# CleanDiffuserTeam/CleanDiffuser

Hardware: AMD Instinct MI355X
Metric: denoised trajectories/sec @ (B=256,H=32,D=23) 20-step DDIM (higher is better)
Workload: dtype f32; 1 GPU; BASELINE configs[1]: JannerUNet1d Diffuser H=32 D=23, 20-step DDIM, global B=256, whole DiscreteDiffusionSDE.sample() call as a pipeline makes it (initial draw inside); batch_per_gpu=256, global_batch=256, horizon=32, dim=23, sample_steps=20, world_size=1, parallelism=batch-sharded x1; the only data-path collective is the all-gather of the result

## Files before the change

### cleandiffuser_amd/csrc/cdx_unet2.hip

```cpp
#include <hip/hip_runtime.h>
#include <stdint.h>
#include <string.h>

#include "../../include/cdx.h"
#include "cdx_act.h"
#include "cdx_ops2.h"
#include "cdx_step.h"

typedef float f32x4 __attribute__((ext_vector_type(4)));
typedef const int __attribute__((address_space(4))) cint;
#pragma clang diagnostic push
#pragma clang diagnostic ignored "-Wold-style-cast"
static __device__ __forceinline__ const cint* as_const(const int* p) { return (const cint*)p; }
#pragma clang diagnostic pop

void cdx_set_err(const char* msg);

template <int NWV> struct WG {
    static constexpr int THREADS = NWV * 64;
    static constexpr int PF = NWV == 8 ? 8 : 16;
    static constexpr int OPW = CDX2_HDR_WORDS + NWV * CDX2_ITEM_WORDS;
};

namespace {
// ... 42 lines not shown
    switch (id) {
        case 2: return mish2(x);
        case 3: {
            const float z = fabsf(x) * 0.70710678118654752f;
            const float t = __builtin_amdgcn_rcpf(fmaf(0.3275911f, z, 1.0f));
            const float poly = t * fmaf(t, fmaf(t, fmaf(t, fmaf(t, 1.061405429f, -1.453152027f), 1.421413741f), -0.284496736f), 0.254829592f);
            return 0.5f * x * (1.0f + copysignf(1.0f - poly * __expf(-z * z), x));
        }
        case 4: return cdx_act_leaky(x);
        case 5: return cdx_act_silu(x);
        case 6: return cdx_act_relu(x);
        case 7: return 0.5f * x * (1.0f + tanhf(0.7978845608028654f * (x + 0.044715f * x * x * x)));
        case 9: return tanhf(x);
        default: return x;
    }
}

struct M16 {
    static constexpr int COLS = 16, KSTEP = 16;
    static __device__ __forceinline__ int col(int lane) { return lane & 15; }
    static __device__ __forceinline__ int koff(int lane) { return 4 * (lane >> 4); }
    static __device__ __forceinline__ int drow(int lane) { return 4 * (lane >> 4); }
    static __device__ __forceinline__ f32x4 mfma(float a, float b, f32x4 c) {
        return __builtin_amdgcn_mfma_f32_16x16x4f32(a, b, c, 0, 0, 0);
    }
};
struct M4 {
    static constexpr int COLS = 4, KSTEP = 4;
    static __device__ __forceinline__ int col(int lane) { return lane & 3; }
    static __device__ __forceinline__ int koff(int) { return 0; }
    static __device__ __forceinline__ int drow(int lane) { return 4 * (lane >> 2); }
    static __device__ __forceinline__ f32x4 mfma(float a, float b, f32x4 c) {
        return __builtin_amdgcn_mfma_f32_4x4x1f32(a, b, c, 0, 0, 0);
    }
};

typedef const cdx_unet2_launch __attribute__((address_space(4))) KArg;

#pragma clang diagnostic push
#pragma clang diagnostic ignored "-Wold-style-cast"
static __device__ __forceinline__ const KArg* kernarg() { return (const KArg*)__builtin_amdgcn_kernarg_segment_ptr(); }
#pragma clang diagnostic pop

struct Geom {
    int l_cols, cstride, ostride, sstride, stage;
    int gsh, grows;
};

struct Item { int woff, nq, tap, cc, part, col0, pad, ooff, src, sstr, ccn; };

__device__ __forceinline__ Item make_item(int woff, int nq, int tc, int part, int col0, int po, int ss, int ccn) {
    return Item{woff, nq, tc & 255, tc >> 8, part, col0, po & 255, po >> 8, ss & 0xffff, ss >> 16, ccn};
}
__device__ __forceinline__ Item load_item(const cint* it) {
    return make_item(it[CDX2_I2_WOFF], it[CDX2_I2_NQ], it[CDX2_I2_TAPCC], it[CDX2_I2_PART], it[CDX2_I2_COL0],
                     it[CDX2_I2_PADOOFF], it[CDX2_I2_SRCSTR], it[CDX2_I2_CCN]);
}

#define CDX2_DW(vd, k) __builtin_amdgcn_readlane((vd), (k))
template <int NWV>
__device__ __forceinline__ int load_desc(const int* __restrict__ ops, int op, int lane, int wave) {
    const int w = lane < CDX2_HDR_WORDS ? lane : CDX2_HDR_WORDS + wave * CDX2_ITEM_WORDS + (lane & (CDX2_ITEM_WORDS - 1));
    return ops[op * WG<NWV>::OPW + w];
}
__device__ __forceinline__ Item inline_item(int vd) {
    const int b = CDX2_HDR_WORDS;
    return make_item(CDX2_DW(vd, b + CDX2_I2_WOFF), CDX2_DW(vd, b + CDX2_I2_NQ), CDX2_DW(vd, b + CDX2_I2_TAPCC),
                     CDX2_DW(vd, b + CDX2_I2_PART), CDX2_DW(vd, b + CDX2_I2_COL0), CDX2_DW(vd, b + CDX2_I2_PADOOFF),
                     CDX2_DW(vd, b + CDX2_I2_SRCSTR), CDX2_DW(vd, b + CDX2_I2_CCN));
}

__device__ __forceinline__ void stamp(unsigned long long* slot, int tid) {
    if (slot && tid == 0) *slot = __builtin_amdgcn_s_memtime();
}

typedef unsigned u32x4 __attribute__((ext_vector_type(4)));
#define CDX2_N_CUS 256
#define CDX2_GETREG_XCC_ID ((3 << 11) | 20)
static __device__ __forceinline__ int mul24i(int a, int b) { return __mul24(a, b); }
static __device__ __forceinline__ int wave_of(int tid) { return __builtin_amdgcn_readfirstlane(tid >> 6); }
#pragma clang diagnostic push
#pragma clang diagnostic ignored "-Wold-style-cast"
struct WStream {
    __amdgpu_buffer_rsrc_t rs;
    int lane16;
    __device__ __forceinline__ WStream(const float* wblob, int lane)
        : rs(__builtin_amdgcn_make_buffer_rsrc((void*)wblob, 0, 0x7fffffff, 0x00020000)), lane16(lane * 16) {}
    __device__ __forceinline__ f32x4 load(int woff, int q) const {
        return __builtin_bit_cast(f32x4, __builtin_amdgcn_raw_buffer_load_b128(rs, lane16, woff * 4 + q * 1024, 0));
    }
};
#pragma clang diagnostic pop

template <int PF> struct Ring { f32x4 rec[PF]; };

template <class M, int NT, int T, int NWV, bool PROF, bool GRP = false>
__device__ __forceinline__ void conv_kloop(const Geom& g, const float* __restrict__ wblob, int vd, const cint* ops,
                                           Item it, int n_items, float* __restrict__ lds, int tf, int lane, int wave,
                                           Ring<WG<NWV>::PF>& ring, unsigned long long* prof, int tune) {
    constexpr int PF = WG<NWV>::PF, NW = NWV;
    constexpr int BD = NWV == 4 ? ((M::KSTEP == 4 && NT * T == 1) ? 8 : 4)
                                : (NT * T == 1 ? (M::KSTEP == 4 ? 8 : 4) : (NT * T == 2 ? 4 : 2));
    constexpr int NA = NWV == 4 ? 4 : ((M::KSTEP == 4 && NT == 1) ? 4 : 2);
    static_assert(PF % BD == 0, "operand ring must divide the weight ring");
    const int ptid = (wave == 0 && lane == 0) ? 0 : 1;
    for (int item = wave; item < n_items; item += NW) {
        if (item != wave) it = load_item(ops + CDX2_DW(vd, CDX2_W2_ITEMS) + (item - NW) * CDX2_ITEM_WORDS);
        const int nq = it.nq, ccn = it.ccn;
        int cc = it.cc;
        int cur[NT], tstep[NT], mcol[NT];
#pragma unroll
        for (int nt = 0; nt < NT; ++nt) {
            mcol[nt] = it.col0 + nt * M::COLS + M::col(lane);
            const bool valid = mcol[nt] < g.l_cols;
            int mrow = mul24i(mcol[nt], g.cstride);
            if (GRP && g.grows) mrow = mul24i(mcol[nt] >> g.gsh, g.grows) + mul24i(mcol[nt] & ((1 << g.gsh) - 1), g.cstride);
            const int row = valid ? mrow - it.pad + CDX2_HALO2 + it.tap : 0;
            cur[nt] = it.src + __mul24(row, it.sstr) + M::koff(lane) + cc * M::KSTEP;
            tstep[nt] = (valid ? it.sstr : 0) - ccn * M::KSTEP;
        }
        if (PROF && prof && item == 0) { asm volatile("" ::"s"(nq), "v"(cur[0])); stamp(prof + 4, ptid); }
        f32x4 acc[T][NT][NA];
#pragma unroll
        for (int t = 0; t < T; ++t)
#pragma unroll
            for (int nt = 0; nt < NT; ++nt)
#pragma unroll
                for (int j = 0; j < NA; ++j) acc[t][nt][j] = (f32x4){0.f, 0.f, 0.f, 0.f};

        const WStream ws(wblob, lane);
        const int woff = it.woff;
#define CDX2_WLOAD(q) ws.load(woff, (q))
        f32x4 wr[PF];
        if (item == wave) {
#pragma unroll
            for (int u = 0; u < PF; ++u) wr[u] = ring.rec[u];
        } else {
#pragma unroll
            for (int u = 0; u < PF; ++u) wr[u] = CDX2_WLOAD(u);
        }
        f32x4 bq[BD][T][NT];
        auto fetch = [&](f32x4 (&bv)[T][NT]) {
#pragma unroll
            for (int t = 0; t < T; ++t)
#pragma unroll
                for (int nt = 0; nt < NT; ++nt) bv[t][nt] = *reinterpret_cast<const f32x4*>(lds + t * tf + cur[nt]);
        };
        auto advance = [&]() {
#pragma unroll
            for (int nt = 0; nt < NT; ++nt) cur[nt] += M::KSTEP;
            if (++cc == ccn) {
                cc = 0;
#pragma unroll
                for (int nt = 0; nt < NT; ++nt) cur[nt] += tstep[nt];
            }
        };
        const bool aligned = (M::KSTEP == 4 || GRP) && (ccn % PF) == 0 && (it.cc % PF) == 0 && nq >= 2 * PF;
        if (aligned) {
#pragma unroll
            for (int j = 0; j < BD - 1; ++j)
// ... 43 lines not shown
                cc0 = wrap ? 0 : cc0 + PF;
#pragma unroll
                for (int nt = 0; nt < NT; ++nt) rbn[nt] = rb[nt] + PF * M::KSTEP * 4 + (wrap ? tstep[nt] * 4 : 0);
#pragma unroll
                for (int u = 0; u < PF; ++u) {
                    const int ua = u + BD - 1;
#pragma unroll
                    for (int t = 0; t < T; ++t)
#pragma unroll
                        for (int nt = 0; nt < NT; ++nt)
                            bq[ua % BD][t][nt] = *reinterpret_cast<const f32x4*>(
                                ldsb + (ua < PF ? rb[nt] : rbn[nt]) + t * tf * 4 + (ua % PF) * M::KSTEP * 4);
#pragma unroll
                    for (int j = 0; j < 4; ++j)
#pragma unroll
                        for (int t = 0; t < T; ++t)
#pragma unroll
                            for (int nt = 0; nt < NT; ++nt)
                                acc[t][nt][j % NA] = M::mfma(wr[u][j], bq[u % BD][t][nt][j], acc[t][nt][j % NA]);
                    if (u > 0) refill(u - 1, qi + u - 1 + PF);
                    else if (qi > 0) refill(PF - 1, qi - 1 + PF);
                    if (NWV == 4 || T >= 2) __builtin_amdgcn_sched_barrier(0);
                }
#pragma unroll
                for (int nt = 0; nt < NT; ++nt) rb[nt] = rbn[nt];
            }
            cc = cc0 + BD - 2;
#pragma unroll
            for (int nt = 0; nt < NT; ++nt) cur[nt] = rb[nt] / 4 + (BD - 2) * M::KSTEP;
        }
        for (; qi < nq; qi += PF) {
#pragma unroll
            for (int u = 0; u < PF; ++u) {
                if (qi + u >= nq) break;
                chunk(wr[u], u, qi + u + BD - 1 < nq);
                const int q = qi + u - 1 + PF;
                if (q >= PF && q < nq) refill((u + PF - 1) % PF, q);
            }
        }
        if (NWV == 8) __builtin_amdgcn_s_setprio(0);
        if (PROF && prof && item == 0) { asm volatile("" ::"v"(acc[0][0][0][0]), "v"(acc[0][0][1][0])); stamp(prof + 6, ptid); }
#pragma unroll
        for (int t = 0; t < T; ++t)
#pragma unroll
            for (int nt = 0; nt < NT; ++nt) {
                if (mcol[nt] < g.l_cols) {
                    const int n = mul24i(mcol[nt], g.ostride) + it.ooff;
                    f32x4 dd = acc[t][nt][0];
                    if (NA == 2) dd += acc[t][nt][NA - 1];
                    if (NA == 4) dd = (acc[t][nt][0] + acc[t][nt][1]) + (acc[t][nt][NA / 2] + acc[t][nt][NA - 1]);
                    *reinterpret_cast<f32x4*>(lds + t * tf + g.stage + it.part + mul24i(n, g.sstride) + M::drow(lane)) = dd;
                }
            }
    }
}

struct EpiDesc {
    int flags, c_out, l_out, coutp, sstride, ksplit, dst, dstride, res, rstride, shift, nk;
    int save, savestr, stats, dst2, d2stride;
    int kpost;
    float inv_cnt;
    float odiv;
    int cgreal4;
};
template <bool BWD>
__device__ __forceinline__ EpiDesc decode_epi(int vd) {
    EpiDesc e;
    e.flags = CDX2_DW(vd, CDX2_W2_FLAGS); e.c_out = CDX2_DW(vd, CDX2_W2_COUT); e.l_out = CDX2_DW(vd, CDX2_W2_LOUT);
    e.coutp = CDX2_DW(vd, CDX2_W2_COUTP); e.sstride = CDX2_DW(vd, CDX2_W2_SSTRIDE); e.ksplit = CDX2_DW(vd, CDX2_W2_KSPLIT);
    e.dst = CDX2_DW(vd, CDX2_W2_DST); e.dstride = CDX2_DW(vd, CDX2_W2_DST_STRIDE); e.res = CDX2_DW(vd, CDX2_W2_RES);
    e.rstride = CDX2_DW(vd, CDX2_W2_RES_STRIDE); e.shift = CDX2_DW(vd, CDX2_W2_CG4_SHIFT); e.nk = CDX2_DW(vd, CDX2_W2_NK);
    e.inv_cnt = __int_as_float(CDX2_DW(vd, CDX2_W2_INV_CNT));
    e.kpost = CDX2_DW(vd, CDX2_W2_KPOST);
    e.odiv = BWD ? 1.0f : __int_as_float(CDX2_DW(vd, CDX2_W2_ODIV));
    e.cgreal4 = BWD ? 0 : CDX2_DW(vd, CDX2_W2_CGREAL4);
    e.save = e.savestr = e.stats = e.dst2 = e.d2stride = 0;
    if (BWD && (e.flags & (CDX2_F2_SAVE | CDX2_F2_GNBWD))) {
        e.save = CDX2_DW(vd, CDX2_W2_SAVE); e.savestr = CDX2_DW(vd, CDX2_W2_SAVE_STRIDE); e.stats = CDX2_DW(vd, CDX2_W2_STATS);
        e.dst2 = CDX2_DW(vd, CDX2_W2_DST2); e.d2stride = CDX2_DW(vd, CDX2_W2_DST2_STRIDE);
    }
    return e;
}

struct EpiParams { f32x4 bi, ga, be, em, pb, sc; };

__device__ __forceinline__ void half_sum2(float& a, float& b, int lane) {
    a = dpp_add<0xB1>(a);  b = dpp_add<0xB1>(b);
    a = dpp_add<0x4E>(a);  b = dpp_add<0x4E>(b);
    a = dpp_add<0x141>(a); b = dpp_add<0x141>(b);
    a = dpp_add<0x140>(a); b = dpp_add<0x140>(b);
    const int ia = __builtin_bit_cast(int, a), ib = __builtin_bit_cast(int, b);
    const float a0 = __builtin_bit_cast(float, __builtin_amdgcn_readlane(ia, 0)), a1 = __builtin_bit_cast(float, __builtin_amdgcn_readlane(ia, 16));
    const float a2 = __builtin_bit_cast(float, __builtin_amdgcn_readlane(ia, 32)), a3 = __builtin_bit_cast(float, __builtin_amdgcn_readlane(ia, 48));
    const float b0 = __builtin_bit_cast(float, __builtin_amdgcn_readlane(ib, 0)), b1 = __builtin_bit_cast(float, __builtin_amdgcn_readlane(ib, 16));
    const float b2 = __builtin_bit_cast(float, __builtin_amdgcn_readlane(ib, 32)), b3 = __builtin_bit_cast(float, __builtin_amdgcn_readlane(ib, 48));
    a = lane < 32 ? a0 + a1 : a2 + a3;
    b = lane < 32 ? b0 + b1 : b2 + b3;
}

struct Pub { float* tile; float tag; int vbase, coutp; bool on; };
template <int NK, bool BWD, bool COND = false, bool MLP = false, bool PUBLISH = false>
__device__ __forceinline__ void epilogue(float* __restrict__ tl, const EpiParams& P, const EpiDesc& e, int stage, int c, int pos0,
                                         int pstep, int li, int nv, int lane, int grp, float* __restrict__ ws, const Pub* pub = nullptr) {
    f32x4 v[NK];
    bool ok[NK];
#pragma unroll
// ... 1048 lines not shown
```

### cleandiffuser_amd/engine/program2.py

```python
import os
from dataclasses import dataclass, field
from typing import Dict, List, Optional, Tuple

import numpy as np
import torch
import torch.nn as nn

from .consts import (GN_EPS, MODE_16X16, MODE_4X4, _conv1d_eff, _convT1d_eff, _fbits, slot_stride, supports_janner)

HDR_WORDS = 32
ITEM2_WORDS = 8
NW2 = 4
NW2_MAX = 8
RING2 = 16
RING2_NW8 = 8
GROUPS2 = 8
MAX_NK2 = 4
HALO2 = 2
MIN_SLICE = int(os.environ.get("CDX_UNET2_MIN_SLICE", "3"))
FUSE_SKIP = os.environ.get("CDX_UNET2_FUSE_SKIP", "1") != "0"
FUSE_MAX_RECORDS = int(os.environ.get("CDX_UNET2_FUSE_MAX", "100"))
SPLIT_MIN_RECORDS = int(os.environ.get("CDX_UNET2_SPLIT_MIN", "8"))

(W2_KIND, W2_FLAGS, W2_COUT, W2_LOUT, W2_LCOLS, W2_CSTRIDE, W2_OSTRIDE, W2_MODE, W2_NT, W2_NITEMS, W2_ITEMS, W2_DST,
 W2_DST_STRIDE, W2_SSTRIDE, W2_KSPLIT, W2_BOFF, W2_GAMMA, W2_BETA, W2_EMB, W2_RES, W2_RES_STRIDE, W2_CG4_SHIFT, W2_INV_CNT,
 W2_NK, W2_COUTP, W2_SAVE, W2_SAVE_STRIDE, W2_STATS, W2_DST2, W2_DST2_STRIDE, W2_KPOST, W2_PBIAS) = range(32)
KIND2_CONV, KIND2_HEAD, KIND2_LOADX, KIND2_LOADC = 0, 1, 2, 3
W2_ITEM0 = 32


def op_words(nw: int) -> int:
    return HDR_WORDS + ITEM2_WORDS * nw


def ring_depth(nw: int) -> int:
    return {4: RING2, 8: RING2_NW8}[nw]
I2_WOFF, I2_NQ, I2_TAPCC, I2_PART, I2_COL0, I2_PADOOFF, I2_SRCSTR, I2_CCN = range(8)

F2_GN, F2_EMB, F2_RES, F2_PRED, F2_SAVE, F2_GNBWD, F2_DUAL, F2_SAVE_GLOBAL, F2_FILM = 1, 2, 4, 8, 16, 32, 64, 128, 256
F2_COLNORM, F2_BIAS_EMB, F2_OUT_DIV = 512, 1024, 2048
F2_ACT_SHIFT = 12
W2_ODIV = 26
W2_XG = 28
XG_XCHG, XG_GOP, XG_TRAJ = 1 << 16, 1 << 17, 1 << 18
W2_GMAP = 25
GROUP_MIN_BYTES = None


def group_min_bytes() -> int:
    return GROUP_MIN_BYTES if GROUP_MIN_BYTES is not None else int(os.environ.get("CDX_UNET2_GROUP_MIN_KB", "400")) * 1024
W2_CGREAL4 = 29


def pad32(c: int) -> int:
    n = (c + 31) // 32
    return 32 * (1 << (n - 1).bit_length())


@dataclass
class Act:
    length: int
    chans: int
    uid: int
    off: int = -1
    persistent: bool = False
    halo: int = HALO2
    in_global: bool = False
    gcap: bool = False
    gk: int = 1

    @property
    def stride(self):
        return slot_stride(self.chans)

    @property
    def sub_floats(self):
        return (self.length + 2 * self.halo) * self.stride

    @property
    def floats(self):
        return self.sub_floats * self.gk

    @property
    def data_off(self):
        return self.off + self.halo * self.stride


@dataclass
class Program2:
    ops: np.ndarray
    ops_buffer: np.ndarray
    blob: torch.Tensor
    traj_floats: int
    x_off: int
    x_stride: int
    pred_off: int
    pred_stride: int
    prev_off: int
    stage_off: int
    horizon: int
    dim: int
    emb_dim: int
    n_emb: int
    embtab: Dict[str, int] = field(default_factory=dict)
    macs_per_forward: int = 0
    n_conv: int = 0
    meta: dict = field(default_factory=dict)
    nw: int = NW2
    embtabs: List[dict] = field(default_factory=list)
    grad_off: int = -1
    grad_stride: int = 0
    ws_floats: int = 0
    compact: bool = False

    def lds_bytes(self, traj_per_wg: int) -> int:
        return 4 * self.traj_floats * traj_per_wg


def _records(w_eff: torch.Tensor, mode: int) -> Tuple[torch.Tensor, int]:
    c_out, taps, cs = w_eff.shape
    rows, kch = (16, 16) if mode == MODE_16X16 else (64, 4)
    n_ct = -(-c_out // rows)
    csp = -(-cs // kch) * kch
    wp = torch.zeros(n_ct * rows, taps, csp, device=w_eff.device, dtype=torch.float32)
    wp[:c_out, :, :cs] = w_eff
    cc = csp // kch
    if mode == MODE_16X16:
        wp = wp.reshape(n_ct, 16, taps, cc, 4, 4).permute(0, 2, 3, 4, 1, 5)
    else:
        wp = wp.reshape(n_ct, 64, taps, cc, 4).permute(0, 2, 3, 1, 4)
    return wp.reshape(n_ct, taps * cc, 64, 4).contiguous(), cc


def _source_records(w: torch.Tensor, srcs: List["Act"], mode: int) -> List[Tuple[torch.Tensor, int]]:
    los = [sum(a.chans for a in srcs[:i]) for i in range(len(srcs))]
    return [_records(w[:, :, lo:lo + a.chans], mode) for a, lo in zip(srcs, los)]


def _slice_edges(n: int, k: int, ring: int) -> List[int]:
    al = ring if n >= 2 * ring * k else 1
    return [min(n, (j * n // k + al // 2) // al * al) for j in range(k)] + [n]


def _deal_over_simds(items: list, item_src: List[int], nw: int):
    load, free, place = [0] * 4, [[sm, sm + 4] for sm in range(4)], {}
    for idx in sorted(range(nw), key=lambda t: -items[t][I2_NQ]):
        sm = min((q for q in range(4) if free[q]), key=lambda q: load[q])
        place[free[sm].pop(0)] = idx
        load[sm] += items[idx][I2_NQ]
    return [items[place[w]] for w in range(nw)], [item_src[place[w]] for w in range(nw)]


@dataclass
class _Stream:
    src: int
    recs: torch.Tensor
    ccn: int
    pad: int
    post: bool


@dataclass
class _ConvView:
    c_out: int
    l_out: int
    phases: list
    l_cols: int
    mode: int
    rows: int
    cols: int
    nt: int
    n_rt: int
    n_cg: int
    my_rts: List[int]
    gop: bool = False
    xg: int = 0

    def __post_init__(self):
        self.coutp = pad32(self.c_out)
        self.tiles = len(self.my_rts) * self.n_cg * len(self.phases)
        self.sstride = (len(self.my_rts) * self.rows + 4) if self.gop else self.coutp + 4
        self.l_stage = self.l_cols if self.gop else self.l_out
        self.rt0 = self.my_rts[0] if self.gop else 0


class _Builder2:
    def __init__(self, device, nw: int = NW2):
        if nw not in (NW2, NW2_MAX):
            raise ValueError(f"v2 programs are compiled for {NW2} or {NW2_MAX} waves, not {nw}")
        self.device = device
        self.nw = nw
        self.ops: List[List[int]] = []
        self.op_acts: List[dict] = []
        self.op_item_src: List[List[int]] = []
        self.op_items: List[list] = []
        self.chunks: List[torch.Tensor] = []
        self.blob_len = 0
        self.acts: List[Act] = []
        self.stage = 0
        self.macs = 0
        self.n_emb = 0
        self.n_stats = 0
        self.max_stage = 1 << 30
        self.alias_residual = False
        self.wrap_live: List[Act] = []
        self.keep_to_end: List[Act] = []
        self.save_global = False
        self.ws_floats = 0
        self.allow_4x4 = True
        self.fuse_max = FUSE_MAX_RECORDS
        self.member = (0, 1)
        self.xchg_floats = 0
        self.grouped = False
        self.group_on = True

    def add(self, t: torch.Tensor, pad_to: int = 4) -> int:
        t = t.detach().to(device=self.device, dtype=torch.float32).reshape(-1)
        off = self.blob_len
        pad = (-t.numel()) % pad_to
        if pad:
            t = torch.cat([t, torch.zeros(pad, device=self.device)])
        self.chunks.append(t)
        self.blob_len += t.numel()
        return off

    def act(self, length: int, chans: int, persistent=False, halo: int = HALO2) -> Act:
        a = Act(length, chans, len(self.acts), persistent=persistent, halo=halo)
        k = self.member[1]
        a.gcap = bool(self.grouped and k > 1 and not persistent and halo == HALO2 and length & (length - 1) == 0 and k * length <= 16)
        self.acts.append(a)
        return a

    def save_slot(self, length: int, chans: int) -> Act:
        a = self.act(length, chans, halo=0)
        if self.save_global:
            a.in_global, a.persistent = True, True
            a.off = self.ws_floats
            self.ws_floats += (a.floats + 3) // 4 * 4
        return a

    def emb_slot(self, c_out: int, film: bool = False) -> int:
        off = self.n_emb
        self.n_emb += pad32(c_out) * (2 if film else 1)
        return off

    def stats_slot(self) -> int:
        off = self.n_stats
        self.n_stats += GROUPS2
        return off

    def conv(self, srcs: List[Act], dst: Act, w_eff: torch.Tensor, bias: Optional[torch.Tensor], *, stride=1, pad=0,
             transposed=False, phases=None, gn: Optional[nn.Module] = None, emb_off: int = -1, res: Optional[Act] = None,
             pred: bool = False, save: Optional[Tuple[Act, int]] = None, bwd: Optional[dict] = None,
             extra: Optional[List[dict]] = None, film: bool = False, act: Optional[int] = None, col_norm: bool = False,
             bias_row: int = -1, out_div: Optional[float] = None, cg_real: int = 0):
        c_out, _, c_in = w_eff.shape
        assert c_in == sum(a.chans for a in srcs) and dst.chans == c_out and 1 <= len(srcs) <= 2
        extra = list(extra or [])
        groupable = phases is None and not transposed and stride == 1 and not col_norm
        phases, l_cols, cstride, ostride = self._geometry(srcs, dst.length, w_eff, stride, pad, transposed, phases)
        v = self._member_view(srcs, dst, w_eff, extra, res, phases, l_cols, groupable=groupable, cuttable=bwd is None and save is None)
        if len(phases) == 1:
            plan = self._plan_single_phase(v, srcs, extra, stride)
            if plan is None:
                return False
        else:
# ... 41 lines not shown
        return mode, rows, cols, nt, -(-c_out // rows), -(-l_cols // (nt * cols))

    def _member_view(self, srcs: List[Act], dst: Act, w_eff: torch.Tensor, extra: List[dict], res: Optional[Act], phases, l_cols: int, *,
                     groupable: bool, cuttable: bool) -> _ConvView:
        c_out, l_out = dst.chans, dst.length
        mem, ksp = self.member
        coutp, cgw = pad32(c_out), pad32(c_out) // GROUPS2
        ex_srcs = [a for ex in extra for a in ex["srcs"]]
        w_bytes = 4 * (w_eff.numel() + sum(ex["w_eff"].numel() for ex in extra))
        gop = (groupable and self.grouped and self.group_on and ksp > 1 and cuttable
               and dst.gcap and all(a.gcap and a.length == l_out for a in list(srcs) + ex_srcs) and (res is None or res.gcap)
               and w_bytes >= group_min_bytes())
        if gop:
            _, rows, _, _, n_rt, n_cg = shape = self._tile_shape(ksp * l_out, c_out)
            lo_c, hi_c = mem * n_rt // ksp * rows, (mem + 1) * n_rt // ksp * rows
            if not (n_rt % ksp or n_cg != 1 or coutp != c_out or lo_c % cgw or hi_c % cgw or GROUPS2 % ksp or -(-(cgw // 4 * l_out) // 32) > 2):
                self.xchg_floats = max(self.xchg_floats, ksp * l_out * coutp)
                for a in list(srcs) + ex_srcs + [dst] + ([res] if res is not None else []):
                    a.gk = ksp
                return _ConvView(c_out, l_out, phases, ksp * l_out, *shape, list(range(mem * n_rt // ksp, (mem + 1) * n_rt // ksp)),
                                 gop=True, xg=(lo_c // cgw) | ((hi_c // cgw) << 8) | XG_XCHG | XG_GOP)
        mode, rows, _, _, n_rt, n_cg = shape = self._tile_shape(l_cols, c_out)
        my_rts, xg = list(range(n_rt)), 0
        k_chunks = sum(-(-a.chans // (16 if mode == MODE_16X16 else 4)) for a in srcs) * phases[0][0].shape[1]
        worth = k_chunks * n_rt * n_cg / self.nw >= SPLIT_MIN_RECORDS
        if (ksp > 1 and not self.grouped and self.group_on and worth and len(phases) == 1 and n_rt > 1 and cuttable
                and (n_rt % ksp == 0 or ksp % n_rt == 0)):
            cand = list(range(mem * n_rt // ksp, (mem + 1) * n_rt // ksp)) if n_rt >= ksp else [mem * n_rt // ksp]
            lo_c, hi_c = cand[0] * rows, (cand[-1] + 1) * rows
            if lo_c % cgw == 0 and hi_c % cgw == 0:
                my_rts, xg = cand, (lo_c // cgw) | (min(hi_c // cgw, GROUPS2) << 8) | (1 << 16)
                self.xchg_floats = max(self.xchg_floats, l_out * coutp)
        return _ConvView(c_out, l_out, phases, l_cols, *shape, my_rts, xg=xg)

    def _slice_counts(self, v: _ConvView, streams: List[_Stream], n_main: int, fusing: bool):
        nw, ring = self.nw, ring_depth(self.nw)
        n_first = nw // v.tiles if v.tiles < nw else 1
        post = [i for i, st in enumerate(streams) if st.post]
        budget = max(len(streams), n_first)
        if v.gop:
            budget = n_first + len(post)
            if os.environ.get("CDX_DBG_LONE") == "1":
                budget = 1 + len(post)
        per = [1] * len(streams)
        n_of = [st.recs.shape[1] for st in streams]
        while sum(per) < budget and (sum(per) + 1) * v.l_stage * v.sstride <= self.max_stage:
            cand = [i for i in range(len(streams)) if n_of[i] // (per[i] + 1) >= MIN_SLICE]
            if not cand:
                break
            per[max(cand, key=lambda i: n_of[i] / per[i])] += 1
        if fusing and max(n_of[i] / per[i] for i in range(n_main)) > self.fuse_max:
            return None
        single_round, uneven = False, {}
        if v.gop and post:
            main = [i for i, st in enumerate(streams) if not st.post]
            uneven_on = os.environ.get("CDX_UNET2_UNEVEN_CUT", "1") != "0"
            if uneven_on and len(main) == 1 and n_first - len(post) >= 2 and n_of[main[0]] >= 2 * ring * (n_first - len(post)):
                per = [1] * len(streams)
                per[main[0]] = n_first - len(post)
                single_round = True
            elif uneven_on and len(main) == 1 and n_first == 2 and n_of[main[0]] >= 4 * ring and n_of[main[0]] % (2 * ring) == 0:
                per[main[0]] = 2
                uneven[main[0]] = [n_of[main[0]] // 2 - ring, n_of[main[0]]]
                spare = budget - 2 - sum(per[i] for i in post)
                for i in sorted(post, key=lambda i: -n_of[i]):
                    while spare < 0 and per[i] > 1:
                        per[i] -= 1
                        spare += 1
        return per, uneven, single_round

    def _plan_single_phase(self, v: _ConvView, srcs: List[Act], extra: List[dict], stride: int):
        w, ppad, _ = v.phases[0]
        all_srcs, pbias = list(srcs), None
        streams = [_Stream(all_srcs.index(a), r, ccn, ppad, False) for a, (r, ccn) in zip(srcs, _source_records(w, srcs, v.mode))]
        for ex in extra:
            w2 = ex["w_eff"]
            assert w2.shape[0] == v.c_out and w2.shape[2] == sum(a.chans for a in ex["srcs"]) and stride == 1
            if ex["pad"] > HALO2 or (w2.shape[1] - 1 - ex["pad"]) > HALO2:
                raise ValueError("extra conv reaches past the halo rows")
            for a, (r, ccn) in zip(ex["srcs"], _source_records(w2, ex["srcs"], v.mode)):
                if a not in all_srcs:
                    all_srcs.append(a)
                streams.append(_Stream(all_srcs.index(a), r, ccn, ex["pad"], bool(ex.get("post"))))
            if ex.get("post"):
                pb = ex.get("bias")
                pbias = (pbias if pbias is not None else torch.zeros(v.c_out, device=self.device)) + \
                    (pb.detach().to(self.device) if pb is not None else 0)
            else:
                assert ex.get("bias") is None, "bias of a summed extra conv: fold it into the main bias"
        counts = self._slice_counts(v, streams, len(srcs), bool(extra))
        if counts is None:
            return None
        per, uneven, single_round = counts
        self.macs += sum(v.c_out * v.l_out * ex["w_eff"].shape[1] * ex["w_eff"].shape[2] for ex in extra)
        order = [i for i, st in enumerate(streams) if not st.post] + [i for i, st in enumerate(streams) if st.post]
        kpost = sum(per[i] for i, st in enumerate(streams) if st.post)
        ksplit = sum(per) - kpost
        items, item_src, ks = [], [], 0
        for i in order:
            st, n, k = streams[i], streams[i].recs.shape[1], per[i]
            woff = self.add(st.recs.contiguous())
            edge = [0] + uneven[i] if i in uneven else _slice_edges(n, k, ring_depth(self.nw))
            for j in range(k):
                q0, q1 = edge[j], edge[j + 1]
                for tile in range(v.n_rt * v.n_cg):
                    rt, cgi = tile % v.n_rt, tile // v.n_rt
                    if rt not in v.my_rts:
                        continue
                    items.append([woff + (rt * n + q0) * 256, q1 - q0, (q0 // st.ccn) | ((q0 % st.ccn) << 8),
                                  ks * v.l_stage * v.sstride + (rt - v.rt0) * v.rows, cgi * v.nt * v.cols, st.pad | (0 << 8), 0, st.ccn])
                    item_src.append(st.src)
                ks += 1
        if single_round and len(items) == self.nw:
            items, item_src = _deal_over_simds(items, item_src, self.nw)
        return items, item_src, ksplit, kpost, pbias, all_srcs

    def _plan_phases(self, v: _ConvView, srcs: List[Act]):
        nw, ring = self.nw, ring_depth(self.nw)
        per_src = max(1, (nw // v.tiles if v.tiles < nw else 1) // len(srcs))
        ph_segs = [_source_records(w, srcs, v.mode) for w, _, _ in v.phases]
        per = [min([per_src] + [max(1, segs[si][0].shape[1] // MIN_SLICE) for segs in ph_segs]) for si in range(len(srcs))]
        while sum(per) > len(srcs) and sum(per) * v.l_out * v.sstride > self.max_stage:
            per[per.index(max(per))] -= 1
        ph_info = []
        for (w, ppad, ooff), segs in zip(v.phases, ph_segs):
            seg_n = [r.shape[1] for r, _ in segs]
            cuts, base = [], 0
            for si, (n, k) in enumerate(zip(seg_n, per)):
                edge = _slice_edges(n, k, ring)
                cuts += [(base + edge[j], base + edge[j + 1], si, base) for j in range(k)]
                base += n
            woff = self.add(torch.cat([r for r, _ in segs], dim=1).contiguous())
            ph_info.append(dict(segs=segs, nqt=sum(seg_n), cuts=cuts, woff=woff, pad=ppad, ooff=ooff))
        ksplit = max(len(pi["cuts"]) for pi in ph_info)
        items, item_src = [], []
        for ks in range(ksplit):
            for tile in range(v.n_rt * v.n_cg):
                rt, cgi = tile % v.n_rt, tile // v.n_rt
                for pi in ph_info:
                    q0, q1, si, sbase = pi["cuts"][ks]
                    ccn = pi["segs"][si][1]
                    items.append([pi["woff"] + (rt * pi["nqt"] + q0) * 256, q1 - q0, ((q0 - sbase) // ccn) | (((q0 - sbase) % ccn) << 8),
                                  ks * v.l_out * v.sstride + rt * v.rows, cgi * v.nt * v.cols, pi["pad"] | (pi["ooff"] << 8), 0, ccn])
                    item_src.append(si)
        if any(len(pi["cuts"]) != ksplit for pi in ph_info):
            raise ValueError("phases with different K-slice counts are not supported (stale partial tiles)")
        return items, item_src, ksplit, 0, None, list(srcs)

    def _epilogue_words(self, words: dict, v: _ConvView, dst: Act, all_srcs: List[Act], bias: Optional[torch.Tensor], pbias, *, gn, bwd,
                        save, emb_off, film, res, pred, bias_row, act, col_norm, cg_real, out_div):
        c_out, l_out, coutp, kpost = v.c_out, v.l_out, v.coutp, words[W2_KPOST]
        if bias_row >= 0:
            assert bias is None, "a table-row bias replaces the static one (fold it into the row)"
            words[W2_BOFF] = bias_row
        else:
            words[W2_BOFF] = self.add(_padded(bias if bias is not None else torch.zeros(c_out, device=self.device), coutp))
        if kpost:
            words[W2_PBIAS] = self.add(_padded(pbias, coutp))
        cg, cg4 = coutp // GROUPS2, coutp // GROUPS2 // 4
        if cg4 & (cg4 - 1) or cg4 > 32:
            raise ValueError(f"C_out {c_out}: the epilogue partitions at most 1024 channels (8 lane groups x 32 float4 lanes)")
        nk = -(-(cg4 * l_out) // 32)
        if nk > MAX_NK2:
            raise ValueError(f"epilogue: {cg4 * l_out} float4 items per group > {32 * MAX_NK2} (horizon too long for v2)")
        words[W2_CG4_SHIFT], words[W2_NK] = cg4.bit_length() - 1, nk
        flags, reads, writes = 0, list(all_srcs), [dst]
# ... 591 lines not shown
    x = b.act(horizon, d, persistent=True)
    blocks, raw_rows = _lower_half_janner_grad(b, clf, horizon, x, None, forward_only=True)
    emb = _emb_table_spec(b, clf, blocks, dev, raw_rows=raw_rows)
    out = b.op_acts[b.head_index]["dst"]
    prog = _finalize2(b, [emb], x, out, horizon, d, clf.emb_dim, max_lds_bytes, [])
    prog.meta["cls_first"], prog.meta["head_op"] = 0, b.head_index
    return prog


def _finalize2(b: "_Builder2", nets_emb: List[dict], x: Act, pred: Act, horizon: int, d: int, emb_dim: int, max_lds_bytes: int,
               persistent: List[Act], grad: Optional[Act] = None, compact: bool = False) -> Program2:
    nw = b.nw
    off = 0
    if compact:
        x.persistent = False
        b.wrap_live.append(x)
        if b.op_acts[0]["srcs"][0] is not x:
            raise ValueError("compact programs expect the state slot to be read by op 0 only")
    else:
        x.off, off = off, off + x.floats
    for a in persistent:
        a.off, off = off, off + a.floats
    prev_off = -4
    if not compact:
        prev_off, off = off, off + (horizon * d + 3) // 4 * 4
    stats_off, off = off, off + (b.n_stats + 3) // 4 * 4
    stage_off, off = off, off + (b.stage + 3) // 4 * 4
    top = (b.plan_arena(off) + 3) // 4 * 4
    if top * 4 > max_lds_bytes:
        raise ValueError(f"LDS plan needs {top * 4} B > {max_lds_bytes} B per trajectory")
    for op in b.ops:
        op[W2_STATS] += stats_off
    tail, cursor = [], len(b.ops) * op_words(nw)
    for op, items in zip(b.ops, b.op_items):
        for j, rec in enumerate(items[:nw]):
            op[W2_ITEM0 + j * ITEM2_WORDS: W2_ITEM0 + (j + 1) * ITEM2_WORDS] = rec
        op[W2_ITEMS] = cursor
        tail += [w for rec in items[nw:] for w in rec]
        cursor += len(items[nw:]) * ITEM2_WORDS
    ops = np.asarray(b.ops, dtype=np.int32)
    ops_buffer = np.concatenate([ops.reshape(-1), np.asarray(tail, dtype=np.int64).astype(np.int32)])
    b.add(torch.zeros(RING2 * 256))
    blob = torch.cat(b.chunks).contiguous()
    return Program2(ops=ops, ops_buffer=ops_buffer, blob=blob, traj_floats=top, x_off=x.data_off,
                    x_stride=x.stride, pred_off=pred.data_off, pred_stride=pred.stride, prev_off=prev_off, stage_off=stage_off,
                    horizon=horizon, dim=d, emb_dim=emb_dim, n_emb=b.n_emb, embtab=nets_emb[0], macs_per_forward=b.macs,
                    n_conv=len(b.ops), meta={"blob_floats": b.blob_len, "stats_off": stats_off}, nw=nw,
                    embtabs=nets_emb, grad_off=-1 if grad is None else grad.data_off, grad_stride=0 if grad is None else grad.stride,
                    compact=compact, ws_floats=((horizon * d + 3) // 4 * 4) if compact else 0)


def _unet_builder(net, nw: int, *, allow_4x4: bool = True, compact: bool = False, max_stage: Optional[int] = None,
                  member: Tuple[int, int] = (0, 1), grouped: bool = False, alias_residual: Optional[bool] = None,
                  what: str = "split / grouped programs") -> _Builder2:
    b = _Builder2(next(net.parameters()).device, nw)
    b.allow_4x4 = allow_4x4
    b.alias_residual = compact if alias_residual is None else alias_residual
    b.member, b.grouped = member, grouped
    if member[1] > 1:
        if compact or nw != NW2_MAX:
            raise ValueError(f"{what}: the 8-wave, state-in-LDS form only")
        b.fuse_max = 1 << 30
    if max_stage is not None:
        b.max_stage = max_stage
    return b


def compile_janner2(net, horizon: int, max_lds_bytes: int = 160 * 1024, allow_4x4: bool = True, nw: int = NW2, compact: bool = False,
                    max_stage: Optional[int] = None, member: Tuple[int, int] = (0, 1), grouped: bool = False,
                    alias_residual: Optional[bool] = None) -> Program2:
    why = supports_janner(net)
    if why is not None:
        raise ValueError(why)
    b = _unet_builder(net, nw, allow_4x4=allow_4x4, compact=compact, max_stage=max_stage, member=member, grouped=grouped,
                      alias_residual=alias_residual)
    d = net.in_dim
    x = b.act(horizon, d, persistent=True)
    t, fc, blocks = _lower_janner(b, net, horizon, x)
    pred = b.act(horizon, d)
    b.conv([t], pred, _conv1d_eff(fc[3]), fc[3].bias, pred=True)
    emb = _emb_table_spec(b, net, blocks, b.device)
    prog = _finalize2(b, [emb], x, pred, horizon, d, net.emb_dim, max_lds_bytes, [], compact=compact)
    prog.meta["xchg_floats"] = b.xchg_floats
    prog.meta["n_gops"] = sum(1 for oa in b.op_acts if oa.get("gop"))
    return prog


def _compile_members(make_member, k: int, grouped: bool, what: Optional[str] = None) -> Program2:
    if k not in (2, 4):
        raise ValueError("group size 2 or 4" if grouped else "split factor 2 or 4")
    if not grouped:
        return _merge_members([make_member(m, None) for m in range(k)], k)
    try:
        members = [make_member(m, False) for m in range(k)]
    except ValueError:
        members = [make_member(m, True) for m in range(k)]
    p0 = _merge_members(members, k)
    p0.meta["group_k"] = k
    del p0.meta["split_k"]
    if p0.meta["n_gops"] == 0:
        raise ValueError(f"{what} streams enough weights to be grouped")
    return p0


def compile_janner2_split(net, horizon: int, k: int, max_lds_bytes: int = 160 * 1024) -> Program2:
    return _compile_members(lambda m, alias: compile_janner2(net, horizon, max_lds_bytes=max_lds_bytes, nw=NW2_MAX, member=(m, k)),
                            k, False)


def _merge_members(members: List[Program2], k: int) -> Program2:
    p0 = members[0]
    n_ops, opw = len(p0.ops), op_words(NW2_MAX)
    for p in members[1:]:
        same = (len(p.ops), p.traj_floats, p.x_off, p.pred_off, p.prev_off, p.stage_off, p.n_emb, p.blob.numel()) == \
               (n_ops, p0.traj_floats, p0.x_off, p0.pred_off, p0.prev_off, p0.stage_off, p0.n_emb, p0.blob.numel())
        if not same or not torch.equal(p.blob, p0.blob):
            raise ValueError("member views of a split program disagree on the LDS plan or the blob")
    ops_all, tails, base = [], [], k * n_ops * opw
    for p in members:
        ops = p.ops.copy()
        tail = p.ops_buffer[n_ops * opw:]
        ops[:, W2_ITEMS] = ops[:, W2_ITEMS] - n_ops * opw + base
        base += tail.size
        ops_all.append(ops)
        tails.append(tail)
    p0.meta["split_k"] = k
    p0.meta["member_ops"] = ops_all
    p0.ops = ops_all[0]
    p0.ops_buffer = np.concatenate([np.concatenate(ops_all).reshape(-1)] + tails).astype(np.int32)
    p0.meta["xchg_floats"] = max(p.meta["xchg_floats"] for p in members)
    if p0.meta["xchg_floats"] == 0:
        raise ValueError("split program: no op of this net streams enough weights to be cut over the members")
    return p0


def compile_janner2_group(net, horizon: int, k: int, max_lds_bytes: int = 160 * 1024) -> Program2:
    return _compile_members(lambda m, alias: compile_janner2(net, horizon, max_lds_bytes=max_lds_bytes, nw=NW2_MAX, member=(m, k),
                                                             grouped=True, alias_residual=alias),
                            k, True, "grouped program: no op of this net")


def compile_guided2(net, clf, horizon: int, max_lds_bytes: int = 160 * 1024, nw: int = NW2_MAX, save_global: bool = False,
                    max_stage: Optional[int] = None, compact: bool = False, member: Tuple[int, int] = (0, 1), grouped: bool = False,
                    alias_residual: Optional[bool] = None) -> Program2:
    why = supports_janner(net)
    if why is not None:
        raise ValueError(why)
    if clf.in_dim != net.in_dim:
        raise ValueError("classifier and denoiser disagree on the state dimension")
    b = _unet_builder(net, nw, compact=compact, max_stage=max_stage, member=member, grouped=grouped, alias_residual=alias_residual,
                      what="grouped / split guided programs")
    b.save_global = save_global
    dev, d = b.device, net.in_dim
    if compact:
        b.ws_floats = (horizon * d + 3) // 4 * 4
    x = b.act(horizon, d, persistent=True)
    pred, grad = b.act(horizon, d), b.act(horizon, d)
    b.keep_to_end += [pred, grad]
    t, fc, blocks = _lower_janner(b, net, horizon, x)
    b.conv([t], pred, _conv1d_eff(fc[3]), fc[3].bias, pred=True)
    n_den = len(b.ops)
    b.group_on = False
    emb_den = _emb_table_spec(b, net, blocks, dev)
    xc = x
    if compact:
        xc = b.act(horizon, d)
        b.load_state(xc)
    cblocks, raw_rows = _lower_half_janner_grad(b, clf, horizon, xc, grad)
    emb_clf = _emb_table_spec(b, clf, cblocks, dev, raw_rows=raw_rows)
    prog = _finalize2(b, [emb_den, emb_clf], x, pred, horizon, d, net.emb_dim, max_lds_bytes, [], grad=grad, compact=compact)
    prog.meta["n_den"] = n_den
    prog.meta["cls_first"], prog.meta["head_op"] = n_den, b.head_index
    prog.ws_floats = b.ws_floats
    prog.meta["xchg_floats"] = b.xchg_floats
    prog.meta["n_gops"] = sum(1 for oa in b.op_acts if oa.get("gop"))
    return prog


def compile_guided2_split(net, clf, horizon: int, k: int, max_lds_bytes: int = 160 * 1024) -> Program2:
    return _compile_members(lambda m, alias: compile_guided2(net, clf, horizon, max_lds_bytes=max_lds_bytes, member=(m, k)), k, False)


def compile_guided2_group(net, clf, horizon: int, k: int, max_lds_bytes: int = 160 * 1024, save_global: bool = False) -> Program2:
    return _compile_members(lambda m, alias: compile_guided2(net, clf, horizon, max_lds_bytes=max_lds_bytes, member=(m, k), grouped=True,
                                                             alias_residual=alias, save_global=save_global),
                            k, True, "grouped guided program: no op of the denoiser")
```

### cleandiffuser_amd/engine/runtime2.py

```python
import ctypes
import os
import warnings
import weakref
from typing import NamedTuple, Optional

import torch

from . import program2 as P2
from . import runtime as R


class CdxUnet2EmbtabArgs(ctypes.Structure):
    _fields_ = [("wblob", ctypes.c_void_p),
                ("emb_dim", ctypes.c_int32), ("hidden", ctypes.c_int32), ("md", ctypes.c_int32), ("n_emb", ctypes.c_int32),
                ("w0", ctypes.c_int32), ("b0", ctypes.c_int32), ("w2", ctypes.c_int32), ("b2", ctypes.c_int32),
                ("w3", ctypes.c_int32), ("b3", ctypes.c_int32),
                ("temb", ctypes.c_void_p), ("n_rows", ctypes.c_int32), ("out", ctypes.c_void_p),
                ("out_ld", ctypes.c_int32), ("col0", ctypes.c_int32),
                ("w4", ctypes.c_int32), ("b4", ctypes.c_int32), ("n_raw", ctypes.c_int32), ("col4", ctypes.c_int32)]


class CdxUnet2Launch(ctypes.Structure):
    _fields_ = [("ops", ctypes.c_void_p), ("wblob", ctypes.c_void_p),
                ("n_ops", ctypes.c_int32), ("traj_floats", ctypes.c_int32), ("traj_per_wg", ctypes.c_int32),
# ... 12 lines not shown
                ("with_backward", ctypes.c_int32), ("ws", ctypes.c_void_p), ("ws_floats", ctypes.c_int32),
                ("compact", ctypes.c_int32), ("prof", ctypes.c_void_p),
                ("emb_per_traj", ctypes.c_int32), ("n_pass", ctypes.c_int32), ("emb_u", ctypes.c_void_p), ("cfg_w", ctypes.c_float),
                ("edm_plan", ctypes.c_int32), ("logp_out", ctypes.c_void_p), ("logp_first_op", ctypes.c_int32),
                ("logp_head_op", ctypes.c_int32), ("ctx", ctypes.c_void_p), ("mlp", ctypes.c_int32),
                ("split_k", ctypes.c_int32), ("xchg_floats", ctypes.c_int32), ("xbuf", ctypes.c_void_p), ("run_if", ctypes.c_void_p),
                ("xerr", ctypes.c_void_p), ("xseq0", ctypes.c_uint32), ("xtick0", ctypes.c_uint32), ("split_group", ctypes.c_int32),
                ("fault", ctypes.c_int32)]


_declared = False


def _lib():
    global _declared
    lib = R.load_library()
    if not _declared:
        lib.cdx_unet2_run.argtypes = [ctypes.POINTER(CdxUnet2Launch), ctypes.c_void_p]
        lib.cdx_unet2_run.restype = ctypes.c_int
        lib.cdx_unet2_embtab.argtypes = [ctypes.POINTER(CdxUnet2EmbtabArgs), ctypes.c_void_p]
        lib.cdx_unet2_embtab.restype = ctypes.c_int
        _declared = True
    return lib


class _Compiled2:
    def __init__(self, prog: Optional[P2.Program2], sig, why: Optional[str] = None):
        self.prog, self.sig, self.why = prog, sig, why
        self.ops_dev = None if prog is None else torch.from_numpy(prog.ops_buffer.copy()).to(prog.blob.device)


_cache = weakref.WeakKeyDictionary()


def _compiled(owner, key, sig, compile_fn, *args) -> _Compiled2:
    per = _cache.setdefault(owner, {})
    hit = per.get(key)
    if hit is not None and hit.sig == sig:
        return hit
    with torch.no_grad():
        try:
            comp = _Compiled2(compile_fn(*args), sig)
        except ValueError as e:
            comp = _Compiled2(None, sig, str(e))
    per[key] = comp
    return comp


def enabled() -> bool:
    return os.environ.get("CDX_UNET2", "1") != "0"


def compiled2(module, horizon: int, nw: int = P2.NW2, compact: bool = False) -> _Compiled2:
    return _compiled(module, ("unet", horizon, nw, bool(compact)), R._signature(module), _compile_unet2, module, horizon, nw, compact)


def _compile_unet2(module, horizon: int, nw: int, compact: bool) -> P2.Program2:
    lower = P2.compile_chiunet2 if R._is_chiunet(module) else P2.compile_janner2
    if compact:
        return lower(module, horizon, nw=nw, compact=True, max_stage=COMPACT_STAGE, max_lds_bytes=(160 * 1024) // 3 // 16 * 16)
    try:
        return lower(module, horizon, nw=nw)
    except ValueError:
        if nw != P2.NW2_MAX or os.environ.get("CDX_UNET2_COMPACT_T1", "1") == "0":
            raise
        return lower(module, horizon, nw=nw, compact=True)


COMPACT_STAGE = 2304


def _structural(module, horizon: int) -> Optional[str]:
    if not enabled():
        return "disabled by CDX_UNET2=0"
    if R._is_chiunet(module):
        if not module.obs_as_global_cond:
            return "ChiUNet1d with local conditioning has no v2 program"
    elif not R._is_janner(module):
        return f"{type(module).__name__} has no v2 program"
    n_down = sum(1 for lvl in module.downs if not isinstance(lvl[-1], torch.nn.Identity))
    if horizon % (1 << n_down) != 0:
        return f"horizon {horizon} not divisible by 2^{n_down}"
    return None


def supported(module, horizon: int) -> Optional[str]:
    why = _structural(module, horizon)
    if why is not None:
        return why
    first = compiled2(module, horizon, DEFAULT_NW)
    return None if first.prog is not None else (compiled2(module, horizon, P2.NW2).why or first.why)


def compact_only(module, horizon: int) -> bool:
    comp = compiled2(module, horizon, DEFAULT_NW)
    return comp.prog is not None and comp.prog.compact


def film_table(comp: _Compiled2, module, t_vec: torch.Tensor, modules=None) -> torch.Tensor:
    prog = comp.prog
    dev = prog.blob.device
    mods = list(modules) if modules is not None else [module]
    assert len(mods) == len(prog.embtabs)
    out = torch.zeros((t_vec.shape[0], prog.n_emb), device=dev, dtype=torch.float32)
    for mod, e in zip(mods, prog.embtabs):
        with torch.no_grad():
            temb = R._f32c(mod.map_noise(t_vec), dev)
# ... 286 lines not shown
        if wait:
            torch.cuda.synchronize(dev)
        if int(word[0]) != 0:
            _modes_off(dev, word)
            if wait:
                word[:] = 0
            raise RuntimeError("cdx_unet2_run (split / grouped program): a member never received a granule; the trajectories of that "
                               "launch were recomputed by the repair launch behind it, and the split / grouped modes are now off for this "
                               f"device (first report: {last_exchange_error[dev]})")


def group_placement(device=None) -> dict:
    device = torch.device("cuda", torch.cuda.current_device()) if device is None else torch.device(device)
    st = _split_bufs.get((device, R._stream_ptr(device)))
    if st is None or "last" not in st:
        return {"workgroups": 0, "groups": 0, "one_xcd_per_group": True, "per_xcd": {}}
    torch.cuda.synchronize(device)
    n_grp, xf, k, tag = st["last"]
    off = n_grp * 4 * xf + 16 * 32
    rec = (st["buf"][off: off + N_CUS].view(torch.int32).cpu().numpy().astype("int64") & 0xffffffff).reshape(n_grp, k)
    live = ((rec >> 4) & 0x0fffffff) == tag
    xcc = rec & 15
    full = live.all(axis=1)
    same = bool(all((xcc[g] == xcc[g][0]).all() for g in range(n_grp) if full[g]))
    per = {}
    for v in xcc[live].tolist():
        per[int(v)] = per.get(int(v), 0) + 1
    return {"workgroups": int(live.sum()), "groups": int(full.sum()), "one_xcd_per_group": same, "per_xcd": per}


def split_factor(batch: int) -> int:
    forced = os.environ.get("CDX_UNET2_SPLIT", "auto")
    if forced == "0" or (forced == "auto" and (os.environ.get("CDX_UNET2_T") or os.environ.get("CDX_UNET2_NW"))):
        return 1
    for k in (4, 2):
        if forced in ("auto", str(k)) and -(-batch // 8) * 8 * k <= N_CUS:
            return k
    return 1


def group_factor(batch: int) -> int:
    forced = os.environ.get("CDX_UNET2_GROUP", "auto")
    if forced == "0" or (forced == "auto" and (os.environ.get("CDX_UNET2_T") or os.environ.get("CDX_UNET2_NW"))):
        return 1
    if not (N_CUS // 2 < batch <= N_CUS) and forced == "auto":
        return 1
    for k in (4, 2):
        if forced in ("auto", str(k)) and -(-batch // (8 * k)) * 8 * k <= N_CUS:
            return k
    return 1


def compiled_group2(module, horizon: int, k: int) -> _Compiled2:
    return _compiled(module, ("group", horizon, k, P2.group_min_bytes()), R._signature(module), P2.compile_janner2_group, module, horizon, k)


def compiled_split2(module, horizon: int, k: int) -> _Compiled2:
    return _compiled(module, ("split", horizon, k), R._signature(module), P2.compile_janner2_split, module, horizon, k)


_emb_bufs = {}


def cond_film_table(comp: _Compiled2, module, t_vec: torch.Tensor, cond: Optional[torch.Tensor], per_sample: bool = False) -> torch.Tensor:
    prog = comp.prog
    dev = prog.blob.device
    e = prog.embtabs[0]
    with torch.no_grad():
        temb = R._f32c(module.map_noise(t_vec), dev)
        if per_sample:
            rows = temb if cond is None else temb + cond
        else:
            rows = (temb[:, None, :] + cond[None, :, :]).reshape(-1, temb.shape[1])
        rows = rows.contiguous()
    n = rows.shape[0]
    key = (dev, R._stream_ptr(dev))
    buf = _emb_bufs.get(key)
    if buf is None or buf.numel() < (n + 2) * prog.n_emb:
        _emb_bufs[key] = buf = torch.zeros((n + 2) * prog.n_emb, device=dev, dtype=torch.float32)
    out = buf[: (n + 2) * prog.n_emb].view(n + 2, prog.n_emb)
    args = CdxUnet2EmbtabArgs(wblob=prog.blob.data_ptr(), emb_dim=e["emb_dim"], hidden=e["hidden"], md=e["md"], n_emb=e["n_emb"],
                              w0=e["w0"], b0=e["b0"], w2=e["w2"], b2=e["b2"], w3=e["w3"], b3=e["b3"],
                              temb=rows.data_ptr(), n_rows=n, out=out.data_ptr(), out_ld=prog.n_emb, col0=e["col0"],
                              w4=e["w4"], b4=e["b4"], n_raw=e["n_raw"], col4=e["col4"])
    R._check(_lib().cdx_unet2_embtab(ctypes.byref(args), R._stream_ptr(dev)), "cdx_unet2_embtab")
    return out


def chi_film_table(comp: _Compiled2, module, t_vec: torch.Tensor, cond: Optional[torch.Tensor], per_sample: bool = False,
                   plan=None) -> torch.Tensor:
    from . import blocks
    prog = comp.prog
    dev = prog.blob.device
    f = prog.meta["chi_film"]
    with torch.no_grad():
        memo = plan.__dict__.setdefault("_memo", {}) if plan is not None else None
        key_t = ("chi_te", str(dev), id(module))
        hit = memo.get(key_t) if memo is not None else None
        if hit is None or hit[0] != comp.sig:
            temb = R._f32c(module.map_noise(t_vec), dev)
            h = blocks.linear(temb, module.map_emb[0].weight, module.map_emb[0].bias, act="mish")
            hit = (comp.sig, blocks.linear(h, module.map_emb[2].weight, module.map_emb[2].bias, act="mish"))
            if memo is not None:
                memo[key_t] = hit
        te = hit[1]
        gce = module.global_cond_encoder
        c_in = cond if cond is not None else torch.zeros((1, gce.in_features), device=dev, dtype=torch.float32)
        ce = blocks.linear(R._f32c(c_in, dev), gce.weight, gce.bias, act="mish")
        cpart = blocks.linear(ce, f["w_c"], f["bias"])
        n_b = cpart.shape[0]
        if per_sample or cond is None:
# ... 406 lines not shown
```

Measured before the change: 71140 trajectories/s.

## Split conv ops into multi-round item schedules and prefetch next item descriptor

Adds an item-rounds lowering mode that cuts main and post streams into more k-slices than waves. Each wave then processes several items in rounds, and the slices are dealt so that light and heavy items pair up, balancing per-wave work. In the kernel, the next item's descriptor is loaded per-lane before the current item's k-loop and broadcast with readlane afterwards, replacing a scalar load at loop top. The mode is on by default for split/group programs and adds extra staging traffic and more item iterations per op.

```diff
diff --git a/cleandiffuser_amd/csrc/cdx_unet2.hip b/cleandiffuser_amd/csrc/cdx_unet2.hip
--- a/cleandiffuser_amd/csrc/cdx_unet2.hip
+++ b/cleandiffuser_amd/csrc/cdx_unet2.hip
@@ -118,10 +118,6 @@
 __device__ __forceinline__ Item make_item(int woff, int nq, int tc, int part, int col0, int po, int ss, int ccn) {
     return Item{woff, nq, tc & 255, tc >> 8, part, col0, po & 255, po >> 8, ss & 0xffff, ss >> 16, ccn};
 }
-__device__ __forceinline__ Item load_item(const cint* it) {
-    return make_item(it[CDX2_I2_WOFF], it[CDX2_I2_NQ], it[CDX2_I2_TAPCC], it[CDX2_I2_PART], it[CDX2_I2_COL0],
-                     it[CDX2_I2_PADOOFF], it[CDX2_I2_SRCSTR], it[CDX2_I2_CCN]);
-}
 
 #define CDX2_DW(vd, k) __builtin_amdgcn_readlane((vd), (k))
 template <int NWV>
@@ -129,12 +125,12 @@
     const int w = lane < CDX2_HDR_WORDS ? lane : CDX2_HDR_WORDS + wave * CDX2_ITEM_WORDS + (lane & (CDX2_ITEM_WORDS - 1));
     return ops[op * WG<NWV>::OPW + w];
 }
-__device__ __forceinline__ Item inline_item(int vd) {
-    const int b = CDX2_HDR_WORDS;
+__device__ __forceinline__ Item lane_item(int vd, const int b) {
     return make_item(CDX2_DW(vd, b + CDX2_I2_WOFF), CDX2_DW(vd, b + CDX2_I2_NQ), CDX2_DW(vd, b + CDX2_I2_TAPCC),
                      CDX2_DW(vd, b + CDX2_I2_PART), CDX2_DW(vd, b + CDX2_I2_COL0), CDX2_DW(vd, b + CDX2_I2_PADOOFF),
                      CDX2_DW(vd, b + CDX2_I2_SRCSTR), CDX2_DW(vd, b + CDX2_I2_CCN));
 }
+__device__ __forceinline__ Item inline_item(int vd) { return lane_item(vd, CDX2_HDR_WORDS); }
 
 __device__ __forceinline__ void stamp(unsigned long long* slot, int tid) {
     if (slot && tid == 0) *slot = __builtin_amdgcn_s_memtime();
@@ -171,7 +167,8 @@
     static_assert(PF % BD == 0, "operand ring must divide the weight ring");
     const int ptid = (wave == 0 && lane == 0) ? 0 : 1;
     for (int item = wave; item < n_items; item += NW) {
-        if (item != wave) it = load_item(ops + CDX2_DW(vd, CDX2_W2_ITEMS) + (item - NW) * CDX2_ITEM_WORDS);
+        const bool has_next = item + NW < n_items;
+        const int vnext = ops[(has_next ? CDX2_DW(vd, CDX2_W2_ITEMS) + item * CDX2_ITEM_WORDS : 0) + (lane & (CDX2_ITEM_WORDS - 1))];
         const int nq = it.nq, ccn = it.ccn;
         int cc = it.cc;
         int cur[NT], tstep[NT], mcol[NT];
@@ -321,6 +318,11 @@
                     *reinterpret_cast<f32x4*>(lds + t * tf + g.stage + it.part + mul24i(n, g.sstride) + M::drow(lane)) = dd;
                 }
             }
+        if (has_next) {
+            int vn = vnext;
+            asm volatile("" : "+v"(vn));
+            it = lane_item(vn, 0);
+        }
     }
 }
 
diff --git a/cleandiffuser_amd/engine/program2.py b/cleandiffuser_amd/engine/program2.py
--- a/cleandiffuser_amd/engine/program2.py
+++ b/cleandiffuser_amd/engine/program2.py
@@ -45,6 +45,15 @@
 XG_XCHG, XG_GOP, XG_TRAJ = 1 << 16, 1 << 17, 1 << 18
 W2_GMAP = 25
 GROUP_MIN_BYTES = None
+
+
+ITEM_ROUNDS = None
+
+
+def item_rounds(runtime_member: bool = False) -> bool:
+    if ITEM_ROUNDS is not None:
+        return bool(ITEM_ROUNDS)
+    return runtime_member and os.environ.get("CDX_UNET2_ITEM_ROUNDS", "1") != "0"
 
 
 def group_min_bytes() -> int:
@@ -149,6 +158,14 @@
         place[free[sm].pop(0)] = idx
         load[sm] += items[idx][I2_NQ]
     return [items[place[w]] for w in range(nw)], [item_src[place[w]] for w in range(nw)]
+
+
+def _deal_rounds(items: list, item_src: List[int], nw: int):
+    if len(items) <= nw or nw != NW2_MAX:
+        return items, item_src
+    order = sorted(range(nw), key=lambda t: items[t][I2_NQ])
+    order = order[:4] + order[:3:-1]
+    return [items[t] for t in order] + items[nw:], [item_src[t] for t in order] + item_src[nw:]
 
 
 @dataclass
@@ -212,6 +229,7 @@
         self.member = (0, 1)
         self.xchg_floats = 0
         self.grouped = False
+        self.item_rounds = False
         self.group_on = True
 
     def add(self, t: torch.Tensor, pad_to: int = 4) -> int:
@@ -359,6 +377,28 @@
         if fusing and max(n_of[i] / per[i] for i in range(n_main)) > self.fuse_max:
             return None
         single_round, uneven = False, {}
+        if self.item_rounds and not v.gop and post and n_first >= 2:
+            main = [i for i, st in enumerate(streams) if not st.post]
+            cut = [0] * len(streams)
+            for i in main:
+                cut[i] = 1
+            while sum(cut) < max(len(main), n_first):
+                cand = [i for i in main if n_of[i] // (cut[i] + 1) >= MIN_SLICE]
+                if not cand:
+                    break
+                cut[max(cand, key=lambda i: n_of[i] / cut[i])] += 1
+            for i in post:
+                cut[i] = max(1, min(4 // v.tiles, n_of[i] // ring))
+
+            def busiest(counts, dealt):
+                nqs = [e[j + 1] - e[j] for i in main + post for e in [_slice_edges(n_of[i], counts[i], ring)]
+                       for j in range(counts[i]) for _ in range(v.tiles)]
+                if dealt:
+                    nqs = [it[I2_NQ] for it in _deal_rounds([{I2_NQ: q} for q in nqs], [0] * len(nqs), nw)[0]]
+                return max(sum(nqs[w::nw]) for w in range(nw))
+            if (sum(cut) <= sum(per) + 2 and sum(cut) * v.l_stage * v.sstride <= self.max_stage
+                    and busiest(cut, True) < busiest(per, False)):
+                return cut, uneven, "rounds"
         if v.gop and post:
             main = [i for i, st in enumerate(streams) if not st.post]
             uneven_on = os.environ.get("CDX_UNET2_UNEVEN_CUT", "1") != "0"
@@ -418,7 +458,9 @@
                                   ks * v.l_stage * v.sstride + (rt - v.rt0) * v.rows, cgi * v.nt * v.cols, st.pad | (0 << 8), 0, st.ccn])
                     item_src.append(st.src)
                 ks += 1
-        if single_round and len(items) == self.nw:
+        if single_round == "rounds":
+            items, item_src = _deal_rounds(items, item_src, self.nw)
+        elif single_round and len(items) == self.nw:
             items, item_src = _deal_over_simds(items, item_src, self.nw)
         return items, item_src, ksplit, kpost, pbias, all_srcs
 
@@ -1116,11 +1158,12 @@
 
 def _unet_builder(net, nw: int, *, allow_4x4: bool = True, compact: bool = False, max_stage: Optional[int] = None,
                   member: Tuple[int, int] = (0, 1), grouped: bool = False, alias_residual: Optional[bool] = None,
-                  what: str = "split / grouped programs") -> _Builder2:
+                  what: str = "split / grouped programs", rounds: Optional[bool] = None) -> _Builder2:
     b = _Builder2(next(net.parameters()).device, nw)
     b.allow_4x4 = allow_4x4
     b.alias_residual = compact if alias_residual is None else alias_residual
     b.member, b.grouped = member, grouped
+    b.item_rounds = item_rounds() if rounds is None else rounds
     if member[1] > 1:
         if compact or nw != NW2_MAX:
             raise ValueError(f"{what}: the 8-wave, state-in-LDS form only")
@@ -1132,12 +1175,22 @@
 
 def compile_janner2(net, horizon: int, max_lds_bytes: int = 160 * 1024, allow_4x4: bool = True, nw: int = NW2, compact: bool = False,
                     max_stage: Optional[int] = None, member: Tuple[int, int] = (0, 1), grouped: bool = False,
-                    alias_residual: Optional[bool] = None) -> Program2:
+                    alias_residual: Optional[bool] = None, rounds: Optional[bool] = None) -> Program2:
     why = supports_janner(net)
     if why is not None:
         raise ValueError(why)
+    if item_rounds() if rounds is None else rounds:
+        try:
+            return _compile_janner2(net, horizon, max_lds_bytes, allow_4x4, nw, compact, max_stage, member, grouped, alias_residual, True)
+        except ValueError:
+            pass
+    return _compile_janner2(net, horizon, max_lds_bytes, allow_4x4, nw, compact, max_stage, member, grouped, alias_residual, False)
+
+
+def _compile_janner2(net, horizon: int, max_lds_bytes: int, allow_4x4: bool, nw: int, compact: bool, max_stage: Optional[int],
+                     member: Tuple[int, int], grouped: bool, alias_residual: Optional[bool], rounds: bool) -> Program2:
     b = _unet_builder(net, nw, allow_4x4=allow_4x4, compact=compact, max_stage=max_stage, member=member, grouped=grouped,
-                      alias_residual=alias_residual)
+                      alias_residual=alias_residual, rounds=rounds)
     d = net.in_dim
     x = b.act(horizon, d, persistent=True)
     t, fc, blocks = _lower_janner(b, net, horizon, x)
@@ -1167,9 +1220,9 @@
     return p0
 
 
-def compile_janner2_split(net, horizon: int, k: int, max_lds_bytes: int = 160 * 1024) -> Program2:
-    return _compile_members(lambda m, alias: compile_janner2(net, horizon, max_lds_bytes=max_lds_bytes, nw=NW2_MAX, member=(m, k)),
-                            k, False)
+def compile_janner2_split(net, horizon: int, k: int, max_lds_bytes: int = 160 * 1024, rounds: Optional[bool] = None) -> Program2:
+    return _compile_members(lambda m, alias: compile_janner2(net, horizon, max_lds_bytes=max_lds_bytes, nw=NW2_MAX, member=(m, k),
+                                                             rounds=rounds), k, False)
 
 
 def _merge_members(members: List[Program2], k: int) -> Program2:
@@ -1198,9 +1251,9 @@
     return p0
 
 
-def compile_janner2_group(net, horizon: int, k: int, max_lds_bytes: int = 160 * 1024) -> Program2:
+def compile_janner2_group(net, horizon: int, k: int, max_lds_bytes: int = 160 * 1024, rounds: Optional[bool] = None) -> Program2:
     return _compile_members(lambda m, alias: compile_janner2(net, horizon, max_lds_bytes=max_lds_bytes, nw=NW2_MAX, member=(m, k),
-                                                             grouped=True, alias_residual=alias),
+                                                             grouped=True, alias_residual=alias, rounds=rounds),
                             k, True, "grouped program: no op of this net")
 
 
diff --git a/cleandiffuser_amd/engine/runtime2.py b/cleandiffuser_amd/engine/runtime2.py
--- a/cleandiffuser_amd/engine/runtime2.py
+++ b/cleandiffuser_amd/engine/runtime2.py
@@ -88,7 +88,7 @@
 
 
 def compiled2(module, horizon: int, nw: int = P2.NW2, compact: bool = False) -> _Compiled2:
-    return _compiled(module, ("unet", horizon, nw, bool(compact)), R._signature(module), _compile_unet2, module, horizon, nw, compact)
+    return _compiled(module, ("unet", horizon, nw, bool(compact), P2.item_rounds()), R._signature(module), _compile_unet2, module, horizon, nw, compact)
 
 
 def _compile_unet2(module, horizon: int, nw: int, compact: bool) -> P2.Program2:
@@ -481,11 +481,15 @@
 
 
 def compiled_group2(module, horizon: int, k: int) -> _Compiled2:
-    return _compiled(module, ("group", horizon, k, P2.group_min_bytes()), R._signature(module), P2.compile_janner2_group, module, horizon, k)
+    rounds = P2.item_rounds(True)
+    return _compiled(module, ("group", horizon, k, P2.group_min_bytes(), rounds), R._signature(module),
+                     lambda m, h, kk: P2.compile_janner2_group(m, h, kk, rounds=rounds), module, horizon, k)
 
 
 def compiled_split2(module, horizon: int, k: int) -> _Compiled2:
-    return _compiled(module, ("split", horizon, k), R._signature(module), P2.compile_janner2_split, module, horizon, k)
+    rounds = P2.item_rounds(True)
+    return _compiled(module, ("split", horizon, k, rounds), R._signature(module),
+                     lambda m, h, kk: P2.compile_janner2_split(m, h, kk, rounds=rounds), module, horizon, k)
 
 
 _emb_bufs = {}
```

New measurement: 71160 trajectories/s, median of 5. About the same (+0.0%).
